# better-flow/better-flow

Measured on AMD Instinct MI355X. Metric: Mevents/s motion-compensated (warp→converged score), 1M-ev slice, 1/2/4/8 GPU, higher is better.
Workload: dtype f64

## Files before the change

better_flow_amd/accel.py:

```python
import ctypes as C
import os

import numpy as np

_DIR = os.path.dirname(os.path.abspath(__file__))
LIB_PATH = os.environ.get("BF_ACCEL_LIB") or os.path.join(_DIR, "libbf_accel.so")
DEBUG_LIB_PATH = os.path.join(_DIR, "debug", "libbf_accel.so")

BF_OK, BF_SKIPPED = 0, 1
BF_ERR_ARG, BF_ERR_HIP, BF_ERR_STATE, BF_ERR_NOCONV, BF_ERR_NODEVICE, BF_ERR_CAPACITY = (
    -1, -2, -3, -4, -5, -6)


class Model(C.Structure):
    _fields_ = [
        ("cx", C.c_double), ("cy", C.c_double), ("dx", C.c_double), ("dy", C.c_double),
        ("rot", C.c_double), ("div", C.c_double), ("cnt", C.c_uint32), ("_pad", C.c_uint32),
        ("total_dx", C.c_double), ("total_dy", C.c_double),
        ("total_rot", C.c_double), ("total_div", C.c_double),
    ]

    def as_dict(self):
        return {k: getattr(self, k) for k, _ in self._fields_ if k != "_pad"}

# ... 215 lines not shown
    "bf_emit_create", "bf_emit_destroy", "bf_emit_reset", "bf_emit_output", "bf_emit_slice", "bf_emit_wait", "bf_emit_release",
    "bf_frame_create", "bf_frame_destroy", "bf_frame_render", "bf_frame_wait", "bf_frame_release", "bf_render_frame",
    "bf_flow_field", "bf_color_flow_img", "bf_flow_frame_create", "bf_flow_frame_destroy", "bf_flow_frame_render",
    "bf_flow_frame_wait", "bf_flow_frame_release", "bf_render_flow_frame",
    "bf_global_hold_field", "bf_global_hold_best", "bf_global_get_flow", "bf_global_flow_field", "bf_global_color_flow_img",
    "bf_global_flow_frame_render", "bf_global_render_flow_frame", "bf_global_emit_slice",
    "bf_segment_opts_default", "bf_segment", "bf_segment_get", "bf_label_image",
    "bf_set_groups", "bf_set_groups_from_segments", "bf_run_groups", "bf_assign_groups",
    "bf_propose_models", "bf_project_groups",
]

BF_FRAME_PPM, BF_FRAME_AVI = 1, 2
BF_FLOW_FRAME_FLO = 4
BF_FLOW_LAST_UPLOADED, BF_FLOW_FIRST_UPLOADED = 0, 1
BF_GLOBAL_HOLD_CELLS, BF_GLOBAL_HOLD_FIELD = 1, 2

_lib = None


def device_numa_node(device=0):
    node = C.c_int32(-1)
    load().bf_device_numa_node(device, C.byref(node))
    return node.value


def bind_thread_to_numa_node(node):
    n = C.c_int32(0)
    rc = load().bf_bind_thread_to_numa_node(node, C.byref(n))
    if rc < 0:
        raise BfError(rc, "bf_bind_thread_to_numa_node(%d)" % node)
# ... 763 lines not shown
```

better_flow_amd/csrc/bf_context.cpp:

```cpp
#include "bf_ctx.h"

std::atomic<int> g_live_ctx[64];

extern "C" {

const char* bf_version(void) { return "bf_accel gfx950 r5"; }

int bf_device_count(int32_t* count) {
    int n = 0;
    hipError_t e = hipGetDeviceCount(&n);
    if (count) *count = (e == hipSuccess) ? n : 0;
    return (e == hipSuccess && n > 0) ? BF_OK : BF_ERR_NODEVICE;
}

int bf_abi_struct_sizes(int32_t* out, int32_t n) {
    const int32_t sz[10] = {(int32_t)sizeof(bf_model),     (int32_t)sizeof(bf_window),
                            (int32_t)sizeof(bf_run_opts),  (int32_t)sizeof(bf_run_info),
                            (int32_t)sizeof(bf_trace_rec), (int32_t)sizeof(bf_profile),
                            (int32_t)sizeof(bf_local_window), (int32_t)sizeof(bf_local_state),
                            (int32_t)sizeof(bf_global_pyramid_opts), (int32_t)sizeof(bf_global_pyramid_info)};
    if (!out) return 10;
    const int32_t m = n < 0 ? 0 : (n < 10 ? n : 10);
    for (int i = 0; i < m; ++i) out[i] = sz[i];
    return m;
// ... 152 lines not shown

int bf_get_stat(bf_ctx* c, const char* key, int64_t* value) {
    if (!c || !key || !value) return BF_ERR_ARG;
    if (!strcmp(key, "scatter_format")) {
        *value = c->use_binned ? c->fmt : -1;
        return BF_OK;
    }
    if (!strcmp(key, "one_kernel")) {
        *value = plan_one_kernel(c) ? 1 : 0;
        return BF_OK;
    }
    if (!strcmp(key, "persistent")) {
        *value = plan_persistent(c) ? 1 : 0;
        return BF_OK;
    }
    if (!strcmp(key, "persist_giveups")) {
        *value = c->persist_giveups;
        return BF_OK;
    }
    const struct { const char* name; int v; } launched[] = {
        {"k1_threads", c->launched.k1_threads}, {"k1_events_per_thread", c->launched.k1_per_thread}, {"k1_head", c->launched.k1_head},
        {"k3_half_scale", c->launched.k3_half_scale}, {"k3_mode", c->launched.k3_mode}, {"k3_capped", c->launched.k3_capped},
        {"bin_rows", c->use_binned ? c->grid.TSR : 0}, {"bin_cols", c->use_binned ? c->grid.TS : 0},
        {"bin_margin", c->use_binned ? c->grid.D : 0}, {"bins", c->use_binned ? c->grid.nbins : 0},
        {"groups_lds", c->groups_lds}, {"groups_per_cu", c->groups_per_cu},
        {"propose_form", c->propose_form}};
    for (const auto& e : launched)
        if (!strcmp(key, e.name)) {
            *value = e.v;
            return BF_OK;
// ... 19 lines not shown
    }
    if (!strcmp(key, "co_schedule")) {
        c->opt_co_schedule = value != 0;
        return BF_OK;
    }
    if (!strcmp(key, "stream_prealloc")) {
        if (!value) return BF_OK;
        HIP_TRY(c, hipSetDevice(c->device));
        const int rc = streaming_setup(c);
        if (rc != BF_OK) return rc;
        for (bf_ctx::UploadSlot& s : c->up.slot) {
            HIP_TRY(c, s.ts.grow((size_t)c->cap_events));
            HIP_TRY(c, s.in16.grow((size_t)c->cap_events * 2));
            HIP_TRY(c, s.noise.grow((size_t)c->cap_events));
        }
        return BF_OK;
    }
    if (!strcmp(key, "sep_update")) {
        if (value < 0 || value > 2) return fail(c, BF_ERR_ARG, "sep_update must be 0 (never), 1 (auto) or 2 (always)");
        c->opt_sep_update = (int)value;
        return BF_OK;
    }
    if (!strcmp(key, "defer_uploads")) {
        if (!value) {
            HIP_TRY(c, hipSetDevice(c->device));
            const int rc = issue_deferred_uploads(c);
            if (rc != BF_OK) return rc;
        }
        c->opt_defer_uploads = value != 0;
        return BF_OK;
// ... 210 lines not shown
```

better_flow_amd/csrc/bf_ctx.h:

```cpp
#pragma once
#pragma clang diagnostic ignored "-Wunused-function"
#include <hip/hip_runtime.h>

#include <atomic>
#include <cerrno>
#include <climits>
#include <cmath>
#include <cstdarg>
#include <cstdio>
#include <cstdlib>
#include <chrono>
#include <cstring>
#include <ctime>
#include <memory>
#include <mutex>
#include <new>
#include <utility>
#include <string>
#include <thread>
#include <vector>

#include "bf_assign.h"
#include "bf_device.h"
#include "bf_kernels.h"
// ... 121 lines not shown
        DevArray<uint8_t> noise;
        EvSet inc;
        HostArray<SliceStats> stats;
        Event copy_done;
        Event staged;
        Event prepared;
        Event inc_free;
        bool staged_valid = false, inc_free_valid = false;
    };
    struct Uploads {
        Stream stream;
        UploadSlot slot[2];
        int head = 0, count = 0;
        UploadSlot& at(int k) { return slot[(head + k) & 1]; }
    } up;
    int opt_sep_update = 1;
    bool opt_defer_uploads = false;
    std::mutex stats_mu;
    const SliceStats* stats_src = nullptr;
    hipEvent_t stats_event = nullptr;
    DevArray<double2> d_nxny, d_uv;
    DevArray<unsigned long long> d_plane[2];
    DevArray<uint32_t> d_cplane[2];
    DevArray<float> d_time, d_gx, d_gy, d_img;
    DevArray<uint32_t> d_count;
    DevArray<MomentAcc> d_acc;
    bool acc_dirty = false;
    DevArray<uint32_t> d_ovf;
    DevArray<unsigned int> d_ticket;
    DevArray<unsigned long long> d_tl;
// ... 87 lines not shown

extern "C" int render_projection_img(bf_ctx* c, int32_t scale, int32_t res_x, int32_t res_y, int32_t show_final, uint8_t* d_img);
extern "C" int render_projection_img_of(bf_ctx* c, const uint32_t* xy, const float2* p, const uint8_t* noise, long long n,
                                        int32_t scale, int32_t res_x, int32_t res_y, int32_t show_final, uint8_t* d_img);
extern "C" int render_color_time_img(bf_ctx* c, int32_t scale, int32_t res_x, int32_t res_y, int32_t show_final, uint8_t* d_bgr);

int ctx_time_img_pass(bf_ctx* c, const char* who);

struct SlicePlan {
    BinGrid grid{}, fgrid{};
    bool binned = false, fused_ok = false, fused_shared = false;
    int fmt = 0, zw = 0;
};
struct RunPlan {
    bool fused = false, binned = false, persist = false;
    bool head_update = false, sep_update = false;
    bool split = false;
    int bin_threads = 0, ev_per_thread = 8;
    bool warm_start = false, prewarp = false, first_warp = false;
    bool quick_warm = false, snap_polled = false;
    double drift_limit = 1e300;
    bool head_like() const { return head_update || sep_update; }
};
SlicePlan plan_slice(const bf_ctx* c, const bf_window& w);
bool plan_one_kernel(const bf_ctx* c);
bool plan_persistent(const bf_ctx* c);
RunPlan plan_run(bf_ctx* c, const bf_run_opts& o);

int streaming_setup(bf_ctx* c);
int issue_deferred_uploads(bf_ctx* c);
// ... 356 lines not shown
```

better_flow_amd/csrc/bf_kernels.h:

```cpp
#pragma once
#include <hip/hip_runtime.h>
#include <hip/hip_ext.h>
#include <stdint.h>
#include <atomic>

#include "bf_device.h"
#include "bf_plan_rules.h"

namespace bf {

constexpr int kHistCopies = 8;
using bf_rules::kBinTileLdsMax;
static_assert(bf_rules::kStencilTileR == kTileR && bf_rules::kStencilTileC == kTileC, "the rules count the stencil kernel's own tiles");
constexpr int kPrepBlocks = 1024;

struct SliceStats {
    int32_t xmin, xmax, ymin, ymax, tmin, tmax;
    long long tsum;
};

struct WarpScatterArgs {
    const uint32_t* xy;
    const int32_t* t;
    float2* p;
// ... 76 lines not shown
    if (raised.load(std::memory_order_acquire) & dev_bit) return hipSuccess;
    for (const void* f : fns) {
        const hipError_t e = hipFuncSetAttribute(f, hipFuncAttributeMaxDynamicSharedMemorySize, kBinTileLdsMax);
        if (e != hipSuccess) return e;
    }
    raised.fetch_or(dev_bit, std::memory_order_release);
    return hipSuccess;
}

void launch_set_state(DevState* st, const DevState& v, hipStream_t s);
void launch_project_dn(const uint32_t* xy, const int32_t* t, float2* p, double2* nxny, const uint32_t* perm, int have_n,
                       const DevState* st, long long n, hipStream_t s);
void launch_final_warp(const WarpScatterArgs& a, hipStream_t s);
void launch_warp_scatter(const WarpScatterArgs& a, bool warp, bool scatter, bool write_n,
                         hipStream_t s);
void launch_prepare(const int32_t* fr_x, const int32_t* fr_y, const int32_t* t_in, uint32_t* xy,
                    int32_t* t_out, float2* p, long long n, long long n_pad, SliceStats* stats,
                    hipStream_t s);
void launch_local_time(const unsigned long long* ts, unsigned long long t0, int32_t* t_out, long long n, hipStream_t s);
void launch_local_time16(const unsigned long long* ts, bool ts32, const uint16_t* row, const uint16_t* col, unsigned long long t0,
                         int32_t* x_out, int32_t* y_out, int32_t* t_out, long long n, hipStream_t s);
void stencil_grid(int R, int C, int* gx, int* gy);
void launch_stencil(const StencilArgs& a, int src, hipStream_t s, int n_cus = 0);
void launch_finish_update(DevState* st, MomentAcc* acc, const uint32_t* ovf_prev, int j, int cur_prev, bf_trace_rec* trace,
                          DevState* snap, hipStream_t s, const uint32_t* lost = nullptr, unsigned long long* snap_seq = nullptr,
                          unsigned long long seq = 0);
void launch_compute_uv(const double2* nxny, double2* uv, long long n, hipStream_t s);
void launch_unpermute(const double2* src, const uint32_t* perm, double2* dst, long long n, hipStream_t s);
void launch_expand_pr(const uint32_t* xy, const float2* p, const uint32_t* perm, double2* pr, long long n,
                      hipStream_t s);
// ... 17 lines not shown
int launch_tile_optimizer(const TileArgs& a, int ntiles, hipStream_t s);
int launch_tile_optimizer_many(const TileArgs* slices, int nslices, int ntiles, int scale, int max_px, uint32_t* counter, int n_cus,
                               hipStream_t s);
void launch_fill_states(DevState* states, const DevState& tmpl, int nt, hipStream_t s);
constexpr int kGroupLdsBudget = 156 * 1024;
int launch_group_sort(const uint32_t* xy, const int32_t* t, const uint32_t* perm_in, long long n, const int32_t* gid, int K,
                      uint32_t* hist, uint32_t* start, uint32_t* cursor, uint32_t* oxy, int32_t* ot, float2* op,
                      uint32_t* operm, hipStream_t s);
void launch_group_boxes(const uint32_t* xy, const uint32_t* perm, const int32_t* gid, const uint32_t* start, long long n, int K,
                        int32_t* box, hipStream_t s);
int launch_group_optimizer(const TileArgs& a, const uint32_t* order, int K, bool warm, uint32_t* counter, int n_cus,
                           hipStream_t s, int* per_cu_out);
void launch_group_rest(const uint32_t* perm, const uint32_t* start, int K, double2* nxny, hipStream_t s);

int bin_kernel_setup();
void launch_stencil_binned(const StencilArgs& a, dim3 grid, hipStream_t s, int n_cus);
void launch_margin_clean(unsigned long long* mplane, const uint32_t* mlist, uint32_t* mcount, int nbins, int mcap, hipStream_t s);
void launch_rebin(const EvSets& sets, int has_perm, long long n, DevState* st, const BinGrid& g,
                  uint16_t* binid, uint32_t* hist_cnt, uint32_t* bin_start,
                  uint32_t* cursor, uint32_t* armed, const WarpParams* prewarp, int pack_limit, hipStream_t s,
                  uint32_t* ftab = nullptr, uint32_t* lost = nullptr);
struct BinScatterArgs {
    EvSets sets;
    const uint32_t* bin_start;
    unsigned long long* slabs;
    uint16_t* cidx;
    uint32_t* chdr;
    int compact;
    unsigned long long* ovf_plane;
    uint32_t* ovf_cplane;
// ... 227 lines not shown
```

better_flow_amd/csrc/bf_kernels.hip:

```cpp
#include <hip/hip_runtime.h>
#include <limits.h>
#include <math.h>

#include "bf_device.h"
#include "bf_device_fns.h"
#include "bf_kernels.h"

namespace bf {

template <bool WARP, bool SCATTER, bool WRITE_N, bool PACKED>
__device__ __forceinline__ void event_body(uint32_t xy, int32_t t, float2& p, bool live,
                                           bool noise, double2* nxny, double2* uv, const uint32_t* perm,
                                           long long slot,
                                           unsigned long long* plane, uint32_t* cplane,
                                           const HotState& st, const WarpParams& wp) {
    const uint32_t fx = xy & 0xffffu, fy = xy >> 16;
    double pr_x = pr_from_p(fx, p.x);
    double pr_y = pr_from_p(fy, p.y);
    if (WARP) {
        double nx, ny;
        warp_products(wp, pr_x, pr_y, t, p, nx, ny);
        pr_x = pr_from_p(fx, p.x);
        pr_y = pr_from_p(fy, p.y);
        if (WRITE_N && live) {
// ... 51 lines not shown
        const uchar4 vn = *reinterpret_cast<const uchar4*>(noise + base);
        z0 = vn.x; z1 = vn.y; z2 = vn.z; z3 = vn.w;
    }
    event_body<WARP, SCATTER, WRITE_N, PACKED>(vxy.x, vt.x, p0, base + 0 < n, z0, nxny, uv, perm, base + 0,
                                               plane, cplane, hs, wp);
    event_body<WARP, SCATTER, WRITE_N, PACKED>(vxy.y, vt.y, p1, base + 1 < n, z1, nxny, uv, perm, base + 1,
                                               plane, cplane, hs, wp);
    event_body<WARP, SCATTER, WRITE_N, PACKED>(vxy.z, vt.z, p2, base + 2 < n, z2, nxny, uv, perm, base + 2,
                                               plane, cplane, hs, wp);
    event_body<WARP, SCATTER, WRITE_N, PACKED>(vxy.w, vt.w, p3, base + 3 < n, z3, nxny, uv, perm, base + 3,
                                               plane, cplane, hs, wp);
    if (WARP) {
        *reinterpret_cast<float4*>(p + base) = make_float4(p0.x, p0.y, p1.x, p1.y);
        *reinterpret_cast<float4*>(p + base + 2) = make_float4(p2.x, p2.y, p3.x, p3.y);
    }
}

__global__ __launch_bounds__(kThreads) void k_project_dn(const uint32_t* __restrict__ xy, const int32_t* __restrict__ t, float2* __restrict__ p,
                                                         double2* __restrict__ nxny, const uint32_t* __restrict__ perm, int have_n,
                                                         const DevState* __restrict__ st, long long n) {
    const long long i = (long long)blockIdx.x * kThreads + threadIdx.x;
    if (i >= n) return;
    const WarpParams wp = st->hot.wp;
    const uint32_t v = xy[i];
    float2 q = p[i];
    const double pr_x = pr_from_p(v & 0xffffu, q.x), pr_y = pr_from_p(v >> 16, q.y);
    const long long o = perm ? (long long)perm[i] : i;
    const double2 old = have_n ? nxny[o] : make_double2(0.0, 0.0);
    const double rx = pr_x - wp.cx, ry = pr_y - wp.cy;
    const double qx = wp.c * rx - wp.s * ry;
// ... 299 lines not shown
                    hipStream_t s) {
    hipLaunchKernelGGL(k_prepare, dim3(kPrepBlocks), dim3(kThreads), 0, s, fr_x, fr_y, t_in, xy,
                       t_out, p, n, n_pad, stats);
}

void stencil_grid(int R, int C, int* gx, int* gy) {
    *gx = (C + kTileC - 1) / kTileC;
    *gy = (R + kTileR - 1) / kTileR;
}

void launch_stencil(const StencilArgs& a, int src, hipStream_t s, int n_cus) {
    int gx, gy;
    stencil_grid(a.R, a.C, &gx, &gy);
    dim3 grid(gx, gy);
    if (src == 3) { launch_stencil_binned(a, grid, s, n_cus); return; }
    if (src == 0) hipLaunchKernelGGL((k_stencil<0, kThreads>), grid, dim3(kThreads), 0, s, a);
    else if (src == 1) hipLaunchKernelGGL((k_stencil<1, kThreads>), grid, dim3(kThreads), 0, s, a);
    else hipLaunchKernelGGL((k_stencil<2, kThreads>), grid, dim3(kThreads), 0, s, a);
}

void launch_compute_uv(const double2* nxny, double2* uv, long long n, hipStream_t s) {
    if (n <= 0) return;
    hipLaunchKernelGGL(k_compute_uv, dim3((unsigned)((n + kThreads - 1) / kThreads)), dim3(kThreads), 0,
                       s, nxny, uv, n);
}

void launch_unpermute(const double2* src, const uint32_t* perm, double2* dst, long long n, hipStream_t s) {
    if (n <= 0) return;
    hipLaunchKernelGGL(k_unpermute, dim3((unsigned)((n + kThreads - 1) / kThreads)), dim3(kThreads), 0, s, src, perm, dst, n);
}
// ... 35 lines not shown
```

better_flow_amd/csrc/bf_plan.cpp:

```cpp
#include "bf_ctx.h"

SlicePlan plan_slice(const bf_ctx* c, const bf_window& w) {
    SlicePlan p;
    const int scale = w.scale;
    BinGrid& g = p.grid;
    const int bin_margin = bf_rules::bin_margin(c->dbg_margin);
    const bf_rules::BinShape shape = bf_rules::bin_shape(c->n, w.scale_img_x, w.scale_img_y, c->n_cus, bin_margin);
    g.TS = shape.TS;
    g.TSR = shape.TSR;
    g.lg = 0;
    while ((1 << g.lg) < g.TS) ++g.lg;
    g.nbc = shape.nbc;
    g.D = shape.D;
    g.L = g.TS + 2 * g.D;
    g.LR = g.TSR + 2 * g.D;
    g.mul_r = (uint32_t)(0x100000000ull / (unsigned)g.TSR) + 1u;
    g.mul_l = (uint32_t)(0x100000000ull / (unsigned)g.L) + 1u;
    g.mul_h = (uint32_t)(0x100000000ull / (unsigned)(g.L / 2 > 0 ? g.L / 2 : 1)) + 1u;
    g.nbr = shape.nbr;
    g.nbins = shape.nbins;
    const bool dense = (double)w.scale_img_x * (double)w.scale_img_y < 12.0 * (double)c->n ||
                       (double)w.scale_img_x * (double)w.scale_img_y <= 9.0e6;
    p.binned = (c->opt_binned == 2 || (c->opt_binned == 1 && dense)) && !c->force_split && !c->has_noise && c->n > 0 &&
               c->cap_events < (1ll << 29) &&
// ... 31 lines not shown
    return p;
}

bool plan_one_kernel(const bf_ctx* c) {
    return c->fused_ok && (!c->opt_co_schedule || c->fused_shared);
}

bool plan_persistent(const bf_ctx* c) {
    return plan_one_kernel(c) && !c->opt_co_schedule && (c->opt_persist == 2 || (c->opt_persist == 1 && c->pending_warp)) &&
           g_live_ctx[c->device & 63].load() == 1 &&
           fused_loop_resident(c->win.scale / 2, c->fgrid.TSR, c->n_cus, c->fgrid.nbr * c->fgrid.nbc);
}

RunPlan plan_run(bf_ctx* c, const bf_run_opts& o) {
    RunPlan p;
    p.fused = plan_one_kernel(c);
    p.binned = c->use_binned || p.fused;
    p.persist = plan_persistent(c);
    if (p.persist && c->persist_skip > 0) { --c->persist_skip; p.persist = false; }
    p.warm_start = c->pending_warp;
    p.prewarp = p.binned && c->pending_warp;
    p.first_warp = c->pending_warp && !p.prewarp;
    if (p.binned) p.drift_limit = c->opt_bin_predict ? (p.persist ? 0.85 : 0.6) * (double)(p.fused ? c->fgrid.D : c->grid.D) : 1e300;
    p.split = c->use_binned && !p.fused && c->fmt == 3;
    p.head_update = p.fused || (p.binned && !c->opt_co_schedule);
    p.sep_update = p.binned && !p.fused && !p.head_update && (c->opt_sep_update == 2 || (c->opt_sep_update == 1 && c->fmt == 2));
    if (p.binned) {
        const bf_rules::ScatterSize k1 = bf_rules::scatter_size(c->fmt, p.head_update, c->grid.nbins, c->n, c->n_cus);
        p.bin_threads = k1.threads;
        p.ev_per_thread = k1.per_thread;
    }
    p.quick_warm = p.warm_start && c->warm_iters_hint < 3 * o.poll_interval;
    p.snap_polled = p.binned && !p.quick_warm;
    return p;
}
```

better_flow_amd/csrc/bf_run.cpp:

```cpp
#include "bf_ctx.h"

namespace {

struct HostTiming {
#ifdef BF_DEBUG_HOOKS
    bool on = [] { static const bool e = getenv("BF_HOST_TIMING") != nullptr; return e; }();
#else
    static constexpr bool on = false;
#endif
    double launch = 0, wait = 0, mark = on ? now() : 0;
    static double now() { return std::chrono::duration<double>(std::chrono::steady_clock::now().time_since_epoch()).count(); }
    void lap(double& into) { if (on) { const double t = now(); into += t - mark; mark = t; } }
};

struct RunLoop {
    bf_ctx* c;
    const RunPlan& p;
    int b0 = 0, buf = 0;
    bool first = true;
    int launched_iters = 0;
    bool prewarp_done = false;
    bf_trace_rec* trace = nullptr;
    bool want_rebin = false;
    int last_rebin_at = 0;
    int skip_rebin_checks = 0;
    int stall_allowance = 0;
    unsigned long long seq_wait = 0;
    bool snap_polled = false;
    bool done = false;
    bool final_done = false;
    DevState fin;
    bf_run_info inf{0, 0, 1.0f, 1.0f, 10000.0f, 10000.0f};
    HostTiming ht;
    DevState* state_of(int j) const { return c->d_state + (p.sep_update ? 0 : (j & 1)); }
    MomentAcc* acc_of(int j) const { return c->d_acc + (size_t)(p.fused ? ((j % 3) + 3) % 3 : (j & 1)) * kAccGroups; }
    uint32_t* ovf_of(int j) const { return c->d_ovf + (((j % 3) + 3) % 3) * kOvfSlotWords; }
    int finish(const DevState& s, bool warped) { fin = s; done = true; final_done = warped; return BF_OK; }
};

int run_begin(bf_ctx* c, const bf_run_opts& o, const RunPlan& p, RunLoop& L) {
    DevState& h = c->hst;
    L.b0 = L.buf = c->cur;
    L.trace = o.trace_cap > 0 ? c->d_trace : nullptr;
    c->p_clean = false;
    c->seg_valid = false;
    c->pending_warp = false;
    h.x_div = h.y_div = 1.0f;
    h.rot_div = h.div_div = 10000.0f;
    h.old_dx = h.old_dy = h.old_rot = h.old_div = 0.f;
// ... 132 lines not shown
        fa.ftab = c->d_ftab;
        fa.st_in = L.state_of(j); fa.st_out = L.state_of(j + 1);
        fa.snap = snap;
        fa.acc_in = L.acc_of(j - 1); fa.acc_out = L.acc_of(j); fa.acc_zero = L.acc_of(j + 1);
        fa.lost = lost_flag(c);
        fa.trace = L.trace;
        fa.nbr = c->fgrid.nbr; fa.nbc = c->fgrid.nbc;
        fa.R = c->win.scale_img_x; fa.C = c->win.scale_img_y;
        fa.j = j;
        fa.warp = warp ? 1 : 0;
        fa.tl = c->d_tl;
        ProfScope ps(c, 0, c->n);
        HIP_TRY(c, launch_fused_pass(fa, c->win.scale / 2, c->fgrid.TSR, c->stream));
        L.inf.launches += 1;
    } else {
        const int buf = L.buf;
        if (p.sep_update) {
            launch_finish_update(L.state_of(j), L.acc_of(j - 1), L.ovf_of(j - 1), j, buf ^ 1, L.trace, snap, c->stream);
            L.inf.launches++;
        }
        if (p.binned) {
            BinScatterArgs ba;
            ba.sets = ev_sets(c);
            ba.bin_start = c->d_bin_start;
            ba.slabs = c->d_slabs;
            ba.cidx = c->d_cidx; ba.chdr = c->d_chdr;
            ba.compact = c->fmt;
            ba.ovf_plane = c->d_plane[buf]; ba.ovf_cplane = c->d_cplane[buf];
            ba.ovf_bits = c->d_ovf_bits[buf]; ba.ovf_pitch = c->ovf_pitch;
            ba.st_in = L.state_of(j); ba.st_out = L.state_of(j + 1);
            ba.acc = p.head_update ? L.acc_of(j - 1) : nullptr;
            ba.ovf_cur = L.ovf_of(j); ba.ovf_prev = L.ovf_of(j - 1);
            ba.snap = snap;
            ba.trace = L.trace;
            ba.g = c->grid;
            ba.cur = buf; ba.j = j;
            ba.tl = c->d_tl ? c->d_tl + 64 * 2 * 16 : nullptr;
            ba.m_cur = c->d_mplane[buf]; ba.m_prev = c->d_mplane[buf ^ 1];
            ba.mlist = c->d_mlist; ba.mcount = c->d_mcount; ba.mcap = c->m_cap;
            ProfScope ps(c, 0, c->n);
            HIP_TRY(c, launch_bin_warp_scatter(ba, warp, p.bin_threads, p.ev_per_thread, c->stream));
            c->launched.k1_threads = p.bin_threads; c->launched.k1_per_thread = p.ev_per_thread; c->launched.k1_head = p.head_update ? 1 : 0;
        } else {
            ProfScope ps(c, 0, c->n);
            launch_warp_scatter(ws_args(c, buf, 1), warp, true, false, c->stream);
        }
        StencilArgs a = st_args(c, buf, 1);
        if (p.binned) {
            a.ovf_bits = c->d_ovf_bits[buf]; a.zero_bits = c->d_ovf_bits[buf ^ 1]; a.ovf_pitch = c->ovf_pitch;
            a.zero_full = j == 0 ? 1 : 0;
            a.st = L.state_of(j + 1);
            a.ovf_cur = L.ovf_of(j); a.ovf_prev = L.ovf_of(j - 1); a.ovf_next = L.ovf_of(j + 1);
            a.tile_bands = (!p.head_update && c->fmt != 2) ? 1 : 0;
        }
        if (p.head_like()) {
            a.acc = L.acc_of(j); a.acc_zero = L.acc_of(j + 1);
        } else if (p.binned) {
            a.acc = c->d_acc;
            a.ticket = c->d_ticket;
            a.st = L.state_of(j);
            a.st_rw = L.state_of(j + 1);
            a.snap = snap;
        } else {
            a.acc = c->d_acc;
            a.ticket = c->d_ticket;
            a.st_rw = c->d_state;
        }
        a.trace = L.trace;
        a.update_mode = 1;
        a.tl = c->d_tl;
        a.tl_launch = j;
        ProfScope ps(c, 1);
        const bool shared_lists = c->opt_co_schedule && c->fmt == 2 && g_live_ctx[c->device & 63].load() > 1;
        const int k3_cus = shared_lists ? 1 : c->n_cus;
        launch_stencil(a, stencil_src(c, p.binned), c->stream, k3_cus);
        if (p.binned) {
            c->launched.k3_half_scale = bf_rules::stencil_half_scale(a.scale);
            c->launched.k3_mode = bf_rules::stencil_mode(a.compact);
            c->launched.k3_capped = bf_rules::stencil_capped(bf_rules::stencil_tiles(a.R, a.C), k3_cus) ? 1 : 0;
        }
        L.inf.launches += 2;
    }
    L.first = false;
    L.buf ^= 1;
    ++L.launched_iters;
    return BF_OK;
}

int enqueue_batch(bf_ctx* c, const bf_run_opts& o, const RunPlan& p, RunLoop& L, int batch) {
    if (p.binned && (batch == 0 || L.want_rebin)) {
        int rc = enqueue_rebin(c, L.state_of(L.launched_iters), c->has_perm, (p.prewarp && batch == 0 && !L.prewarp_done) ? &c->hst.hot.wp : nullptr,
                               p.fused, L.launched_iters);
        if (rc != BF_OK) return rc;
        L.inf.launches += 3;
        L.want_rebin = false;
        L.skip_rebin_checks = 1;
        L.last_rebin_at = L.launched_iters;
        if (p.fused && batch > 0) L.stall_allowance += 3 * o.poll_interval;
    }
// ... 137 lines not shown
    HIP_TRY(c, hipGetLastError());

    const DevState d = L.fin;
    DevState& h = c->hst;
    h = d;
    h.hot.pp = 0; h.hot.redo = 0; h.hot.pend = 0;
    if (p.split) {
        if (d.hot.it > 0) c->m_dirty_plane = L.b0 ^ ((d.hot.it - 1) & 1);
        c->m_unknown = d.rc < 0;
    }
    if (p.binned && !p.fused) {
        h.hot.ovf_cnt[L.b0 ^ (d.hot.it & 1)] = 0;
        h.hot.ovf_cnt[L.b0 ^ (d.hot.it & 1) ^ 1] = d.last_ovf ? 1u : 0u;
    }

    c->cur = p.fused ? L.b0 : (L.b0 ^ (d.hot.it & 1));
    c->trace_valid = d.hot.it < o.trace_cap ? d.hot.it : o.trace_cap;
    L.inf.rc = d.rc;
    L.inf.iterations = d.hot.it;
    L.inf.x_divider = d.x_div; L.inf.y_divider = d.y_div;
    L.inf.rot_divider = d.rot_div; L.inf.div_divider = d.div_div;
    L.inf.rebins = d.hot.rebins;
    L.inf.overflow_events = (int32_t)(d.ovf_total > 0x7fffffffu ? 0x7fffffffu : d.ovf_total);
    if (model_out) *model_out = d.model;
    if (info) *info = L.inf;
    if (d.rc < 0) return fail(c, d.rc, "iteration cap (%d) reached without convergence", o.hard_iter_cap);
    return d.rc;
}

}

// ... 14 lines not shown

int bf_run(bf_ctx* c, const bf_run_opts* opts_in, bf_model* model_out, bf_run_info* info) {
    if (!c) return BF_ERR_ARG;
    if (!c->have_window) return fail(c, BF_ERR_STATE, "bf_run before bf_set_cloud");
    bf_run_opts o;
    if (opts_in) o = *opts_in; else bf_run_opts_default(&o);
    if (o.poll_interval < 1) o.poll_interval = 1;
    HIP_TRY(c, hipSetDevice(c->device));
    const bf_window& w = c->win;

    const bool noise = (w.scale_img_x < w.scale * o.res_x / 15) && (w.scale_img_y < w.scale * o.res_y / 15);
    if (noise) c->all_noise = true;
    if (noise || c->n < (long long)o.min_events) {
        if (model_out) *model_out = c->hst.model;
        if (info) *info = bf_run_info{BF_SKIPPED, 0, 1.0f, 1.0f, 10000.0f, 10000.0f};
        return BF_SKIPPED;
    }

    if (o.trace_cap > 0) HIP_TRY(c, c->d_trace.grow((size_t)o.trace_cap));
    const RunPlan p = plan_run(c, o);
    c->launched = bf_ctx::Launched{};
    RunLoop L{c, p};
    int rc = run_begin(c, o, p, L);
    if (rc == BF_OK && p.persist) rc = run_persistent(c, o, p, L);
    if (rc != BF_OK) return rc;
    L.snap_polled = p.snap_polled && !L.done;
    if (L.snap_polled) {
        *reinterpret_cast<volatile unsigned long long*>(&c->h_state[0]) = 0ull;
        *reinterpret_cast<volatile unsigned long long*>(&c->h_state[0].run_tag) = 0ull;
    }
    for (int batch = 0; !L.done; ++batch) {
        rc = enqueue_batch(c, o, p, L, batch);
        if (rc == BF_OK) rc = L.snap_polled ? wait_snapshot(c, o, p, L)
                            : p.quick_warm ? wait_quick_warm(c, o, p, L, batch) : wait_one_batch_behind(c, o, p, L, batch);
        if (rc != BF_OK) return rc;
    }
    return run_end(c, o, p, L, model_out, info);
}

int bf_run_many(bf_ctx* const* ctxs, int32_t n, const bf_run_opts* opts, bf_model* models_out, bf_run_info* infos_out) {
// ... 27 lines not shown
```

better_flow_amd/csrc/bf_stencil.hip:

```cpp
#include <atomic>
#include <hip/hip_runtime.h>
#include <hip/hip_ext.h>
#include <limits.h>
#include <cstdlib>

#include "bf_device.h"
#include "bf_device_fns.h"
#include "bf_kernels.h"

namespace bf {

constexpr int kStencilSgprs = 74;
constexpr int kTileBandsBit = 0x100;

typedef unsigned int bf_u32x2 __attribute__((ext_vector_type(2)));
__device__ __forceinline__ __amdgpu_buffer_rsrc_t buf_of(const void* base) {
    return __builtin_amdgcn_make_buffer_rsrc(const_cast<void*>(base), 0, -1, 0x00020000);
}
__device__ __forceinline__ unsigned long long buf_ld_u64(__amdgpu_buffer_rsrc_t r, uint32_t thread_bytes, uint32_t uniform_bytes) {
    const bf_u32x2 v = __builtin_amdgcn_raw_buffer_load_b64(r, (int)thread_bytes, (int)uniform_bytes, 0);
    return ((unsigned long long)v.y << 32) | (unsigned long long)v.x;
}

struct K3Pre {
// ... 27 lines not shown
    const int R = pre.R, C = pre.C;
    const int tid = threadIdx.x;
    const double rcp_v = tid < kRcpTab ? c_rcp.v[tid] : 0.0;
    const int lane = tid & 63, wv = __builtin_amdgcn_readfirstlane(tid >> 6);
    int r0, c0;
    if (MODE != 1 && (pre.lg & kTileBandsBit)) {
        const uint32_t gx = (uint32_t)(C + TC - 1) / (uint32_t)TC, gy = (uint32_t)(R + TR - 1) / (uint32_t)TR;
        const uint32_t tile = (uint32_t)bf_rules::tile_of_block((int)blockIdx.x, (int)(gx * gy));
        const uint32_t trow = tile / gx;
        r0 = (int)trow * TR; c0 = (int)(tile - trow * gx) * TC;
    } else {
        r0 = blockIdx.y * TR; c0 = blockIdx.x * TC;
    }
    BinGrid g = a.g;
    g.D = pre.D; g.lg = pre.lg & (kTileBandsBit - 1); g.nbc = pre.nbc; g.nbr = pre.nbr; g.LR = pre.LR; g.L = pre.L; g.TSR = pre.TSR; g.mul_r = pre.mul_r;
    const int bt = hs.bin_tbits;
    const unsigned long long bm = (1ull << bt) - 1ull;
    const bool ovf = sload(a.ovf_cur) != 0;
    const int LLi = g.LR * g.L;

    constexpr bool compact = COMPACT;
    if (compact) {
        static_assert(TH * TW <= PR * PC, "the box plane fits the point plane's LDS");
        for (int idx = tid; idx < TH * TW; idx += NT) s_acc[idx] = 0ull;
        const int br_lo = row_bin(max(r0 - 1 - HS - g.D, 0), g), br_hi = min(row_bin(min(r0 + TR + HS, R - 1) + g.D, g), g.nbr - 1);
        const int bc_lo = max(c0 - 1 - HS - g.D, 0) >> g.lg, bc_hi = min((min(c0 + TC + HS, C - 1) + g.D) >> g.lg, g.nbc - 1);
        constexpr int kMaxBins = 32;
        __shared__ uint32_t s_eoff[kMaxBins + 1];
        __shared__ int2 s_ebin[kMaxBins];
        __shared__ int s_nseg;
        const int ncol = bc_hi - bc_lo + 1;
        const int zw = g.zw, nz = zw ? 3 : 1;
        const int ncand = min((br_hi - br_lo + 1) * ncol * nz, 64);
// ... 110 lines not shown
            we[x][0] = pre.slabs[(uint32_t)(r_off + x_off)];
            if (r_edge || x_edge) we[x][1] = a.m_cur[(uint32_t)(r_moff + x_gc)];
        }
    }
    if (a.check_done && hs.done) return;
#pragma unroll
    for (int k = 0; k < KR; ++k) {
        const int pr = wv + k * NW;
        if (pr < PR) s_acc[pr * PC + lane] = w[k][0] + w[k][1];
    }
#pragma unroll
    for (int x = 0; x < XE; ++x) {
        const int e = lane + 64 * x, pr = wv + (e / XC) * NW;
        if (e < KR * XC && pr < PR) s_acc[pr * PC + 64 + e % XC] = we[x][0] + we[x][1];
    }
    } else {
    static_assert(TR + 2 * H <= 32, "a tile plus halo must fit the smallest bin height (32)");
    const int bl = row_bin(max(r0 - H - g.D, 0), g), bh = row_bin(max(r0 - H + g.D, 0), g);
    const int bl_next = (bl + 1) * g.TSR, bh_next = (bh + 1) * g.TSR;
    const int rb_l0 = bl * g.nbc * LLi - (bl * g.TSR - g.D) * g.L, rb_l1 = rb_l0 + g.nbc * LLi - g.TSR * g.L;
    const int rb_h0 = bh * g.nbc * LLi - (bh * g.TSR - g.D) * g.L, rb_h1 = rb_h0 + g.nbc * LLi - g.TSR * g.L;
    auto col_of = [&](int pc, bool& in, bool& two, int& lo, int& hi) {
        const int gc = c0 - H + pc;
        in = gc >= 0 && gc < C;
        const int bcl = max(gc - g.D, 0) >> g.lg, bch = min((gc + g.D) >> g.lg, g.nbc - 1);
        lo = __mul24(bcl, LLi) - (bcl << g.lg) + g.D + gc;
        hi = __mul24(bch, LLi) - (bch << g.lg) + g.D + gc;
        two = bch > bcl;
    };
    auto row_of = [&](int pr, bool& in, bool& two, int& lo, int& hi) {
// ... 159 lines not shown
        if (wv >= LW && wv < LW + XT && lane < TH) time_px(lane, 64 + (wv - LW), box_at(lane, 64 + (wv - LW)));
    } else {
        if (lane < KT * XT) {
            const int tr = wv + (lane / XT) * NW;
            if (tr < TH) time_px(tr, 64 + lane % XT, box_at(tr, 64 + lane % XT));
        }
    }
    StencilArgs ta = sload(late_args<StencilArgs>(kStencilArgsOffset));
    ta.st = as_global(ta.st); ta.acc = as_global(ta.acc); ta.acc_zero = as_global(ta.acc_zero);
    ta.ovf_cur = as_global(ta.ovf_cur); ta.ovf_prev = as_global(ta.ovf_prev); ta.ovf_next = as_global(ta.ovf_next);
    ta.zero_plane = as_global(ta.zero_plane); ta.zero_cplane = as_global(ta.zero_cplane); ta.zero_bits = as_global(ta.zero_bits);
    ta.ticket = as_global(ta.ticket); ta.st_rw = as_global(ta.st_rw); ta.snap = as_global(ta.snap);
    ta.trace = as_global(ta.trace); ta.tl = as_global(ta.tl);
    __syncthreads();
    tl_stamp(ta.tl, ta.tl_launch, 4);
    const bool do_zero = ta.zero_plane && sload(ta.ovf_prev) != 0;
    static_assert((size_t)PR * PC >= (size_t)(NT / 64) * 192, "the reduction's scratch fits the accumulator plane");
    stencil_tail<TR, TC, NT, false>(ta, s_time, s_red, r0, c0, do_zero, reinterpret_cast<double*>(s_acc));
}

#define BF_K3_PRE_PARAMS const unsigned long long* p_slabs, const DevState* p_st, int p_R, int p_C, int p_D, int p_lg, \
                          int p_nbc, int p_nbr, int p_LR, int p_L, int p_TSR, uint32_t p_mul_r
#define BF_K3_PRE_VALUE K3Pre{p_slabs, p_st, p_R, p_C, p_D, p_lg, p_nbc, p_nbr, p_LR, p_L, p_TSR, p_mul_r}
template <int HS, int MODE, int NT>
__global__ __launch_bounds__(NT) void k_stencil_binned(BF_K3_PRE_PARAMS, StencilArgs a) {
    stencil_binned_body<HS, MODE, NT>(a, BF_K3_PRE_VALUE);
}
template <int HS, int MODE, int NT>
__global__ __launch_bounds__(NT) __attribute__((amdgpu_num_sgpr(kStencilSgprs))) void k_stencil_binned_full(BF_K3_PRE_PARAMS, StencilArgs a) {
    stencil_binned_body<HS, MODE, NT>(a, BF_K3_PRE_VALUE);
}
// ... 11 lines not shown
        else launch_timed(k_stencil_binned_full<HS_, 0, kThreads>, grid, dim3(kThreads), 0, s, BF_K3_PRE, a);                  \
    } else if (a.compact == 3) launch_timed(k_stencil_binned<HS_, 2, kThreads>, grid, dim3(kThreads), 0, s, BF_K3_PRE, a);     \
    else if (a.compact) launch_timed(k_stencil_binned<HS_, 1, kThreads>, grid, dim3(kThreads), 0, s, BF_K3_PRE, a);            \
    else launch_timed(k_stencil_binned<HS_, 0, kThreads>, grid, dim3(kThreads), 0, s, BF_K3_PRE, a)
    switch (bf_rules::stencil_half_scale(a.scale)) {
        case 0: BF_K3(0); break;
        case 1: BF_K3(1); break;
        case 2: BF_K3(2); break;
        case 3: BF_K3(3); break;
        default: BF_K3(4); break;
    }
#undef BF_K3
#undef BF_K3_PRE
}

}
```

include/bf_accel.h:

```cpp
#ifndef BF_ACCEL_H
#define BF_ACCEL_H

#include <stdint.h>

#ifdef __cplusplus
extern "C" {
#endif

#define BF_OK 0
#define BF_SKIPPED 1
#define BF_ERR_ARG (-1)
#define BF_ERR_HIP (-2)
#define BF_ERR_STATE (-3)
#define BF_ERR_NOCONV (-4)
#define BF_ERR_NODEVICE (-5)
#define BF_ERR_CAPACITY (-6)

typedef struct bf_ctx bf_ctx;

typedef struct bf_model {
    double cx, cy, dx, dy, rot, div;
    uint32_t cnt;
    uint32_t _pad;
    double total_dx, total_dy, total_rot, total_div;
// ... 50 lines not shown
              void *hip_stream, bf_ctx **out);

void bf_destroy(bf_ctx *ctx);

const char *bf_last_error(const bf_ctx *ctx);

const char *bf_version(void);

void bf_run_opts_default(bf_run_opts *opts);

int bf_abi_struct_sizes(int32_t *out, int32_t n);

int bf_set_option(bf_ctx *ctx, const char *key, int64_t value);

int bf_get_stat(bf_ctx *ctx, const char *key, int64_t *value);


int bf_upload_events(bf_ctx *ctx, const int32_t *fr_x, const int32_t *fr_y, const int32_t *t_ns,
                     const uint8_t *noise, int64_t n);

int bf_upload_events_device(bf_ctx *ctx, const int32_t *d_fr_x, const int32_t *d_fr_y,
                            const int32_t *d_t_ns, int64_t n);

int bf_host_alloc(bf_ctx *ctx, int64_t bytes, void **out);
int bf_host_free(bf_ctx *ctx, void *ptr);
int bf_upload_events_async(bf_ctx *ctx, const int32_t *fr_x, const int32_t *fr_y, const int32_t *t_ns,
                           int64_t n);
int bf_commit_upload(bf_ctx *ctx);

int bf_set_cloud(bf_ctx *ctx, int32_t scale, int32_t res_x, int32_t res_y, bf_window *window_out);
// ... 345 lines not shown
```

Measured before the change: 217.5.

## Add delta-scatter loop that updates only pixels whose events moved

Adds an iteration mode in which each event's old and new pixel are computed and only events that changed pixel issue atomic subtract/add on a persistent plane, instead of re-scattering all events into a freshly zeroed plane. A new stencil mode reads that flat plane directly through buffer loads, skipping the binned path and its overflow checks. The planner enables it automatically for large packed, co-scheduled, non-noise runs, so it trades per-iteration full rebuilds for a persistent-state scheme that depends on exact integer cancellation and keeps a single plane buffer.

Measured after the change: 240.6, median of 6. 1.11x the previous value.

```diff
diff --git a/better_flow_amd/accel.py b/better_flow_amd/accel.py
--- a/better_flow_amd/accel.py
+++ b/better_flow_amd/accel.py
@@ -253,6 +253,7 @@
 BF_FLOW_FRAME_FLO = 4
 BF_FLOW_LAST_UPLOADED, BF_FLOW_FIRST_UPLOADED = 0, 1
 BF_GLOBAL_HOLD_CELLS, BF_GLOBAL_HOLD_FIELD = 1, 2
+BF_LOOP_ATOMIC, BF_LOOP_BINNED, BF_LOOP_ONE_KERNEL, BF_LOOP_PERSISTENT, BF_LOOP_DELTA = 0, 1, 2, 3, 4
 
 _lib = None
 
diff --git a/better_flow_amd/csrc/bf_context.cpp b/better_flow_amd/csrc/bf_context.cpp
--- a/better_flow_amd/csrc/bf_context.cpp
+++ b/better_flow_amd/csrc/bf_context.cpp
@@ -190,6 +190,10 @@
         *value = plan_persistent(c) ? 1 : 0;
         return BF_OK;
     }
+    if (!strcmp(key, "loop_form")) {
+        *value = c->last_loop;
+        return BF_OK;
+    }
     if (!strcmp(key, "persist_giveups")) {
         *value = c->persist_giveups;
         return BF_OK;
@@ -239,6 +243,11 @@
             HIP_TRY(c, s.in16.grow((size_t)c->cap_events * 2));
             HIP_TRY(c, s.noise.grow((size_t)c->cap_events));
         }
+        return BF_OK;
+    }
+    if (!strcmp(key, "delta_scatter")) {
+        if (value < 0 || value > 2) return fail(c, BF_ERR_ARG, "delta_scatter must be 0 (never), 1 (auto) or 2 (always)");
+        c->opt_delta = (int)value;
         return BF_OK;
     }
     if (!strcmp(key, "sep_update")) {
diff --git a/better_flow_amd/csrc/bf_ctx.h b/better_flow_amd/csrc/bf_ctx.h
--- a/better_flow_amd/csrc/bf_ctx.h
+++ b/better_flow_amd/csrc/bf_ctx.h
@@ -159,6 +159,8 @@
         int head = 0, count = 0;
         UploadSlot& at(int k) { return slot[(head + k) & 1]; }
     } up;
+    int opt_delta = 1;
+    int last_loop = -1;
     int opt_sep_update = 1;
     bool opt_defer_uploads = false;
     std::mutex stats_mu;
@@ -276,6 +278,7 @@
 };
 struct RunPlan {
     bool fused = false, binned = false, persist = false;
+    bool delta = false;
     bool head_update = false, sep_update = false;
     bool split = false;
     int bin_threads = 0, ev_per_thread = 8;
diff --git a/better_flow_amd/csrc/bf_kernels.h b/better_flow_amd/csrc/bf_kernels.h
--- a/better_flow_amd/csrc/bf_kernels.h
+++ b/better_flow_amd/csrc/bf_kernels.h
@@ -114,6 +114,7 @@
 void launch_final_warp(const WarpScatterArgs& a, hipStream_t s);
 void launch_warp_scatter(const WarpScatterArgs& a, bool warp, bool scatter, bool write_n,
                          hipStream_t s);
+void launch_warp_scatter_delta(const WarpScatterArgs& a, hipStream_t s);
 void launch_prepare(const int32_t* fr_x, const int32_t* fr_y, const int32_t* t_in, uint32_t* xy,
                     int32_t* t_out, float2* p, long long n, long long n_pad, SliceStats* stats,
                     hipStream_t s);
@@ -161,6 +162,7 @@
 void launch_group_rest(const uint32_t* perm, const uint32_t* start, int K, double2* nxny, hipStream_t s);
 
 int bin_kernel_setup();
+void launch_stencil_plane(const StencilArgs& a, dim3 grid, hipStream_t s);
 void launch_stencil_binned(const StencilArgs& a, dim3 grid, hipStream_t s, int n_cus);
 void launch_margin_clean(unsigned long long* mplane, const uint32_t* mlist, uint32_t* mcount, int nbins, int mcap, hipStream_t s);
 void launch_rebin(const EvSets& sets, int has_perm, long long n, DevState* st, const BinGrid& g,
diff --git a/better_flow_amd/csrc/bf_kernels.hip b/better_flow_amd/csrc/bf_kernels.hip
--- a/better_flow_amd/csrc/bf_kernels.hip
+++ b/better_flow_amd/csrc/bf_kernels.hip
@@ -89,6 +89,84 @@
         *reinterpret_cast<float4*>(p + base) = make_float4(p0.x, p0.y, p1.x, p1.y);
         *reinterpret_cast<float4*>(p + base + 2) = make_float4(p2.x, p2.y, p3.x, p3.y);
     }
+}
+
+constexpr uint32_t kNoPixel = 0xffffffffu;
+
+__device__ __forceinline__ uint32_t scatter_pixel(uint32_t fx, uint32_t fy, const float2& p, const HotState& st) {
+    const int s = st.scale, hs = s / 2;
+    const int X = trunc_scatter(pr_from_p(fx, p.x) * (double)s + (double)st.x_sh);
+    const int Y = trunc_scatter(pr_from_p(fy, p.y) * (double)s + (double)st.y_sh);
+    if ((X >= st.wsx + hs) || (X < hs) || (Y >= st.wsy + hs) || (Y < hs)) return kNoPixel;
+    return (uint32_t)X * (uint32_t)st.C + (uint32_t)Y;
+}
+
+template <bool PACKED>
+__device__ __forceinline__ void event_delta(uint32_t xy, int32_t t, float2& p, bool live, unsigned long long* plane,
+                                            uint32_t* cplane, const HotState& st) {
+    const uint32_t fx = xy & 0xffffu, fy = xy >> 16;
+    const uint32_t k_old = scatter_pixel(fx, fy, p, st);
+    double nx, ny;
+    warp_products(st.wp, pr_from_p(fx, p.x), pr_from_p(fy, p.y), t, p, nx, ny);
+    const uint32_t k_new = scatter_pixel(fx, fy, p, st);
+    if (!live || k_old == k_new) return;
+    const unsigned long long dt = (unsigned long long)((long long)t - st.tmin);
+    const unsigned long long w = PACKED ? (1ull << st.tbits) + dt : dt;
+    if (k_old != kNoPixel) {
+        (void)__hip_atomic_fetch_add(&plane[k_old], 0ull - w, __ATOMIC_RELAXED, __HIP_MEMORY_SCOPE_AGENT);
+        if (!PACKED) (void)__hip_atomic_fetch_add(&cplane[k_old], 0u - 1u, __ATOMIC_RELAXED, __HIP_MEMORY_SCOPE_AGENT);
+    }
+    if (k_new != kNoPixel) {
+        (void)__hip_atomic_fetch_add(&plane[k_new], w, __ATOMIC_RELAXED, __HIP_MEMORY_SCOPE_AGENT);
+        if (!PACKED) (void)__hip_atomic_fetch_add(&cplane[k_new], 1u, __ATOMIC_RELAXED, __HIP_MEMORY_SCOPE_AGENT);
+    }
+}
+
+template <bool PACKED, int EV>
+__global__ __launch_bounds__(kThreads) void k_warp_scatter_delta(const uint32_t* __restrict__ xy, const int32_t* __restrict__ t,
+                                                                 float2* __restrict__ p, unsigned long long* __restrict__ plane,
+                                                                 uint32_t* __restrict__ cplane, const DevState* __restrict__ st,
+                                                                 long long n, int check_done) {
+    static_assert(EV == 2 || EV == 4, "16-byte stores of the products: two events each");
+    const HotState hs = st->hot;
+    if (check_done == 1 && hs.done) return;
+    const long long base = ((long long)blockIdx.x * kThreads + threadIdx.x) * EV;
+    if (base >= n) return;
+    uint32_t vxy[EV];
+    int32_t vt[EV];
+    float2 q[EV];
+    if (EV == 4) {
+        *reinterpret_cast<uint4*>(vxy) = *reinterpret_cast<const uint4*>(xy + base);
+        *reinterpret_cast<int4*>(vt) = *reinterpret_cast<const int4*>(t + base);
+    } else {
+        *reinterpret_cast<uint2*>(vxy) = *reinterpret_cast<const uint2*>(xy + base);
+        *reinterpret_cast<int2*>(vt) = *reinterpret_cast<const int2*>(t + base);
+    }
+#pragma unroll
+    for (int k = 0; k < EV; k += 2) {
+        const float4 pa = *reinterpret_cast<const float4*>(p + base + k);
+        q[k] = make_float2(pa.x, pa.y);
+        q[k + 1] = make_float2(pa.z, pa.w);
+    }
+#pragma unroll
+    for (int k = 0; k < EV; ++k) event_delta<PACKED>(vxy[k], vt[k], q[k], base + k < n, plane, cplane, hs);
+#pragma unroll
+    for (int k = 0; k < EV; k += 2) {
+        const bf_u32x4 v = {__float_as_uint(q[k].x), __float_as_uint(q[k].y), __float_as_uint(q[k + 1].x), __float_as_uint(q[k + 1].y)};
+        asm volatile("global_store_dwordx4 %0, %1, off sc1" :: "v"(p + base + k), "v"(v) : "memory");
+    }
+}
+
+constexpr int kDeltaEv = 2;
+
+void launch_warp_scatter_delta(const WarpScatterArgs& a, hipStream_t s) {
+    const long long per_block = (long long)kThreads * kDeltaEv;
+    const dim3 grid((unsigned)((a.n + per_block - 1) / per_block));
+    if (grid.x == 0) return;
+    if (a.packed)
+        hipLaunchKernelGGL((k_warp_scatter_delta<true, kDeltaEv>), grid, dim3(kThreads), 0, s, a.xy, a.t, a.p, a.plane, a.cplane, a.st, a.n, a.check_done);
+    else
+        hipLaunchKernelGGL((k_warp_scatter_delta<false, kDeltaEv>), grid, dim3(kThreads), 0, s, a.xy, a.t, a.p, a.plane, a.cplane, a.st, a.n, a.check_done);
 }
 
 __global__ __launch_bounds__(kThreads) void k_project_dn(const uint32_t* __restrict__ xy, const int32_t* __restrict__ t, float2* __restrict__ p,
@@ -418,6 +496,7 @@
     stencil_grid(a.R, a.C, &gx, &gy);
     dim3 grid(gx, gy);
     if (src == 3) { launch_stencil_binned(a, grid, s, n_cus); return; }
+    if (src == 4) { launch_stencil_plane(a, grid, s); return; }
     if (src == 0) hipLaunchKernelGGL((k_stencil<0, kThreads>), grid, dim3(kThreads), 0, s, a);
     else if (src == 1) hipLaunchKernelGGL((k_stencil<1, kThreads>), grid, dim3(kThreads), 0, s, a);
     else hipLaunchKernelGGL((k_stencil<2, kThreads>), grid, dim3(kThreads), 0, s, a);
diff --git a/better_flow_amd/csrc/bf_plan.cpp b/better_flow_amd/csrc/bf_plan.cpp
--- a/better_flow_amd/csrc/bf_plan.cpp
+++ b/better_flow_amd/csrc/bf_plan.cpp
@@ -69,15 +69,20 @@
 
 RunPlan plan_run(bf_ctx* c, const bf_run_opts& o) {
     RunPlan p;
-    p.fused = plan_one_kernel(c);
-    p.binned = c->use_binned || p.fused;
-    p.persist = plan_persistent(c);
+    const double Pdelta = (double)c->win.scale_img_x * (double)c->win.scale_img_y;
+    const bool delta_pays = c->opt_co_schedule && !c->pending_warp && c->opt_binned == 1 && c->opt_fused != 2 && c->use_binned &&
+                            c->fmt == 0 && c->packed && !plan_one_kernel(c) && (double)c->n >= Pdelta && Pdelta < (double)(1u << 28) &&
+                            (o.max_iter <= 0 || o.max_iter >= 200);
+    p.delta = !c->has_noise && c->n > 0 && (c->opt_delta == 2 || (c->opt_delta == 1 && delta_pays));
+    p.fused = !p.delta && plan_one_kernel(c);
+    p.binned = !p.delta && (c->use_binned || p.fused);
+    p.persist = !p.delta && plan_persistent(c);
     if (p.persist && c->persist_skip > 0) { --c->persist_skip; p.persist = false; }
     p.warm_start = c->pending_warp;
     p.prewarp = p.binned && c->pending_warp;
     p.first_warp = c->pending_warp && !p.prewarp;
     if (p.binned) p.drift_limit = c->opt_bin_predict ? (p.persist ? 0.85 : 0.6) * (double)(p.fused ? c->fgrid.D : c->grid.D) : 1e300;
-    p.split = c->use_binned && !p.fused && c->fmt == 3;
+    p.split = p.binned && !p.fused && c->fmt == 3;
     p.head_update = p.fused || (p.binned && !c->opt_co_schedule);
     p.sep_update = p.binned && !p.fused && !p.head_update && (c->opt_sep_update == 2 || (c->opt_sep_update == 1 && c->fmt == 2));
     if (p.binned) {
@@ -86,6 +91,6 @@
         p.ev_per_thread = k1.per_thread;
     }
     p.quick_warm = p.warm_start && c->warm_iters_hint < 3 * o.poll_interval;
-    p.snap_polled = p.binned && !p.quick_warm;
+    p.snap_polled = (p.binned || p.delta) && !p.quick_warm;
     return p;
 }
diff --git a/better_flow_amd/csrc/bf_run.cpp b/better_flow_amd/csrc/bf_run.cpp
--- a/better_flow_amd/csrc/bf_run.cpp
+++ b/better_flow_amd/csrc/bf_run.cpp
@@ -32,7 +32,7 @@
     DevState fin;
     bf_run_info inf{0, 0, 1.0f, 1.0f, 10000.0f, 10000.0f};
     HostTiming ht;
-    DevState* state_of(int j) const { return c->d_state + (p.sep_update ? 0 : (j & 1)); }
+    DevState* state_of(int j) const { return c->d_state + ((p.sep_update || !p.binned) ? 0 : (j & 1)); }
     MomentAcc* acc_of(int j) const { return c->d_acc + (size_t)(p.fused ? ((j % 3) + 3) % 3 : (j & 1)) * kAccGroups; }
     uint32_t* ovf_of(int j) const { return c->d_ovf + (((j % 3) + 3) % 3) * kOvfSlotWords; }
     int finish(const DevState& s, bool warped) { fin = s; done = true; final_done = warped; return BF_OK; }
@@ -195,7 +195,8 @@
         HIP_TRY(c, launch_fused_pass(fa, c->win.scale / 2, c->fgrid.TSR, c->stream));
         L.inf.launches += 1;
     } else {
-        const int buf = L.buf;
+        const bool delta_step = p.delta && !L.first;
+        const int buf = p.delta ? L.b0 : L.buf;
         if (p.sep_update) {
             launch_finish_update(L.state_of(j), L.acc_of(j - 1), L.ovf_of(j - 1), j, buf ^ 1, L.trace, snap, c->stream);
             L.inf.launches++;
@@ -224,9 +225,11 @@
             c->launched.k1_threads = p.bin_threads; c->launched.k1_per_thread = p.ev_per_thread; c->launched.k1_head = p.head_update ? 1 : 0;
         } else {
             ProfScope ps(c, 0, c->n);
-            launch_warp_scatter(ws_args(c, buf, 1), warp, true, false, c->stream);
+            if (delta_step) launch_warp_scatter_delta(ws_args(c, buf, 1), c->stream);
+            else launch_warp_scatter(ws_args(c, buf, 1), warp, true, false, c->stream);
         }
         StencilArgs a = st_args(c, buf, 1);
+        if (delta_step) a.zero_plane = nullptr, a.zero_cplane = nullptr;
         if (p.binned) {
             a.ovf_bits = c->d_ovf_bits[buf]; a.zero_bits = c->d_ovf_bits[buf ^ 1]; a.ovf_pitch = c->ovf_pitch;
             a.zero_full = j == 0 ? 1 : 0;
@@ -246,6 +249,7 @@
             a.acc = c->d_acc;
             a.ticket = c->d_ticket;
             a.st_rw = c->d_state;
+            if (p.delta) a.snap = snap;
         }
         a.trace = L.trace;
         a.update_mode = 1;
@@ -254,7 +258,9 @@
         ProfScope ps(c, 1);
         const bool shared_lists = c->opt_co_schedule && c->fmt == 2 && g_live_ctx[c->device & 63].load() > 1;
         const int k3_cus = shared_lists ? 1 : c->n_cus;
-        launch_stencil(a, stencil_src(c, p.binned), c->stream, k3_cus);
+        const bool plane_k3 = p.delta && c->packed && (unsigned long long)a.R * (unsigned long long)a.C < (1ull << 28);
+        if (plane_k3) a.tile_bands = c->opt_co_schedule ? 1 : 0;
+        launch_stencil(a, plane_k3 ? 4 : stencil_src(c, p.binned), c->stream, k3_cus);
         if (p.binned) {
             c->launched.k3_half_scale = bf_rules::stencil_half_scale(a.scale);
             c->launched.k3_mode = bf_rules::stencil_mode(a.compact);
@@ -263,7 +269,7 @@
         L.inf.launches += 2;
     }
     L.first = false;
-    L.buf ^= 1;
+    if (!p.delta) L.buf ^= 1;
     ++L.launched_iters;
     return BF_OK;
 }
@@ -431,7 +437,7 @@
         h.hot.ovf_cnt[L.b0 ^ (d.hot.it & 1) ^ 1] = d.last_ovf ? 1u : 0u;
     }
 
-    c->cur = p.fused ? L.b0 : (L.b0 ^ (d.hot.it & 1));
+    c->cur = p.fused ? L.b0 : p.delta ? (d.hot.it > 0 ? L.b0 ^ 1 : L.b0) : (L.b0 ^ (d.hot.it & 1));
     c->trace_valid = d.hot.it < o.trace_cap ? d.hot.it : o.trace_cap;
     L.inf.rc = d.rc;
     L.inf.iterations = d.hot.it;
@@ -476,6 +482,7 @@
     if (noise || c->n < (long long)o.min_events) {
         if (model_out) *model_out = c->hst.model;
         if (info) *info = bf_run_info{BF_SKIPPED, 0, 1.0f, 1.0f, 10000.0f, 10000.0f};
+        c->last_loop = -1;
         return BF_SKIPPED;
     }
 
@@ -486,6 +493,7 @@
     int rc = run_begin(c, o, p, L);
     if (rc == BF_OK && p.persist) rc = run_persistent(c, o, p, L);
     if (rc != BF_OK) return rc;
+    c->last_loop = p.delta ? BF_LOOP_DELTA : L.done ? BF_LOOP_PERSISTENT : p.fused ? BF_LOOP_ONE_KERNEL : p.binned ? BF_LOOP_BINNED : BF_LOOP_ATOMIC;
     L.snap_polled = p.snap_polled && !L.done;
     if (L.snap_polled) {
         *reinterpret_cast<volatile unsigned long long*>(&c->h_state[0]) = 0ull;
diff --git a/better_flow_amd/csrc/bf_stencil.hip b/better_flow_amd/csrc/bf_stencil.hip
--- a/better_flow_amd/csrc/bf_stencil.hip
+++ b/better_flow_amd/csrc/bf_stencil.hip
@@ -65,9 +65,10 @@
     }
     BinGrid g = a.g;
     g.D = pre.D; g.lg = pre.lg & (kTileBandsBit - 1); g.nbc = pre.nbc; g.nbr = pre.nbr; g.LR = pre.LR; g.L = pre.L; g.TSR = pre.TSR; g.mul_r = pre.mul_r;
-    const int bt = hs.bin_tbits;
+    const int bt = MODE == 3 ? hs.tbits : hs.bin_tbits;
     const unsigned long long bm = (1ull << bt) - 1ull;
-    const bool ovf = sload(a.ovf_cur) != 0;
+    bool ovf = false;
+    if constexpr (MODE != 3) ovf = sload(a.ovf_cur) != 0;
     const int LLi = g.LR * g.L;
 
     constexpr bool compact = COMPACT;
@@ -208,6 +209,35 @@
         const int e = lane + 64 * x, pr = wv + (e / XC) * NW;
         if (e < KR * XC && pr < PR) s_acc[pr * PC + 64 + e % XC] = we[x][0] + we[x][1];
     }
+    } else if constexpr (MODE == 3) {
+    unsigned long long w[KR], we[XE];
+    const __amdgpu_buffer_rsrc_t plane_buf = buf_of(pre.slabs);
+    const int c_gc = c0 - H + lane;
+    const bool c_in = c_gc >= 0 && c_gc < C;
+#pragma unroll
+    for (int k = 0; k < KR; ++k) {
+        const int pr = wv + k * NW, gr = r0 - H + pr;
+        w[k] = 0ull;
+        if (pr < PR && gr >= 0 && gr < R && c_in) w[k] = buf_ld_u64(plane_buf, (uint32_t)c_gc * 8u, (uint32_t)__mul24(gr, C) * 8u);
+    }
+#pragma unroll
+    for (int x = 0; x < XE; ++x) {
+        const int e = lane + 64 * x;
+        const int pr = wv + (e / XC) * NW, gr = r0 - H + pr, gc = c0 - H + 64 + e % XC;
+        we[x] = 0ull;
+        if (e < KR * XC && pr < PR && gr >= 0 && gr < R && gc >= 0 && gc < C) we[x] = pre.slabs[(uint32_t)(__mul24(gr, C) + gc)];
+    }
+    if (a.check_done && hs.done) return;
+#pragma unroll
+    for (int k = 0; k < KR; ++k) {
+        const int pr = wv + k * NW;
+        if (pr < PR) s_acc[pr * PC + lane] = w[k];
+    }
+#pragma unroll
+    for (int x = 0; x < XE; ++x) {
+        const int e = lane + 64 * x, pr = wv + (e / XC) * NW;
+        if (e < KR * XC && pr < PR) s_acc[pr * PC + 64 + e % XC] = we[x];
+    }
     } else {
     static_assert(TR + 2 * H <= 32, "a tile plus halo must fit the smallest bin height (32)");
     const int bl = row_bin(max(r0 - H - g.D, 0), g), bh = row_bin(max(r0 - H + g.D, 0), g);
@@ -397,7 +427,8 @@
     ta.trace = as_global(ta.trace); ta.tl = as_global(ta.tl);
     __syncthreads();
     tl_stamp(ta.tl, ta.tl_launch, 4);
-    const bool do_zero = ta.zero_plane && sload(ta.ovf_prev) != 0;
+    bool do_zero = ta.zero_plane != nullptr;
+    if constexpr (MODE != 3) do_zero = do_zero && sload(ta.ovf_prev) != 0;
     static_assert((size_t)PR * PC >= (size_t)(NT / 64) * 192, "the reduction's scratch fits the accumulator plane");
     stencil_tail<TR, TC, NT, false>(ta, s_time, s_red, r0, c0, do_zero, reinterpret_cast<double*>(s_acc));
 }
@@ -439,4 +470,18 @@
 #undef BF_K3_PRE
 }
 
-}
+void launch_stencil_plane(const StencilArgs& a, dim3 tiles, hipStream_t s) {
+    const dim3 grid = a.tile_bands ? dim3(tiles.x * tiles.y) : tiles;
+#define BF_K3P(HS_) launch_timed(k_stencil_binned<HS_, 3, kThreads>, grid, dim3(kThreads), 0, s, a.plane, a.st, a.R, a.C, 0, \
+                                 a.tile_bands ? kTileBandsBit : 0, 0, 0, 0, 0, 0, 0u, a)
+    switch (bf_rules::stencil_half_scale(a.scale)) {
+        case 0: BF_K3P(0); break;
+        case 1: BF_K3P(1); break;
+        case 2: BF_K3P(2); break;
+        case 3: BF_K3P(3); break;
+        default: BF_K3P(4); break;
+    }
+#undef BF_K3P
+}
+
+}
diff --git a/include/bf_accel.h b/include/bf_accel.h
--- a/include/bf_accel.h
+++ b/include/bf_accel.h
@@ -88,6 +88,11 @@
 int bf_set_option(bf_ctx *ctx, const char *key, int64_t value);
 
 int bf_get_stat(bf_ctx *ctx, const char *key, int64_t *value);
+#define BF_LOOP_ATOMIC 0
+#define BF_LOOP_BINNED 1
+#define BF_LOOP_ONE_KERNEL 2
+#define BF_LOOP_PERSISTENT 3
+#define BF_LOOP_DELTA 4
 
 
 int bf_upload_events(bf_ctx *ctx, const int32_t *fr_x, const int32_t *fr_y, const int32_t *t_ns,
```
